# VladGavra98/SERL

Hardware: NVIDIA H100
Metric: env_steps_per_sec (higher is better)
Workload: dtype f64 plant + f32 actor

## Files before the change

serl_b200/csrc/gen/plant_rhs_common.h:

```cpp
#define PLANT_NPV 23
PLANT_PV_TABLE = {
  {0x1.6800000000000p+6, 0x0.0p+0, (1.0/0.0), (-1.0/0.0), (1.0/0.0), (-1.0/0.0), 0x1.489db496242c0p-3, 0x1.489db496242c0p-3, 0x1.489db496242c0p-3, 0x1.097333cd78a88p-1, 0x1.10eafeb224ae4p+2, 0x1.99c1db3619942p+2, 0x1.99c1db3619942p+2, 0x1.097333cd78a88p-1, 0x1.10eafeb224ae4p+2, 0x1.10eafeb224ae4p+2, 0x1.10eafeb224ae4p+2, 0x1.097333cd78a88p-1, 0x1.097333cd78a88p-1, 0x1.99c1db3619942p+2, -0x1.097333cd78a88p-1, -0x1.097333cd78a88p-1, -0x1.99c1db3619942p+2},
  {0x1.6800000000000p+6, 0x1.eb851eb851eb8p-5, 0x1.ae147ae147ae1p-1, -0x1.ae147ae147ae1p-1, 0x1.ae147ae147ae1p-1, -0x1.ae147ae147ae1p-1, 0x1.489db496242c0p-3, 0x1.489db496242c0p-3, 0x1.489db496242c0p-3, 0x1.097333cd78a88p-1, 0x1.10eafeb224ae4p+2, 0x1.99c1db3619942p+2, 0x1.99c1db3619942p+2, 0x1.097333cd78a88p-1, 0x1.10eafeb224ae4p+2, 0x1.10eafeb224ae4p+2, 0x1.10eafeb224ae4p+2, 0x1.097333cd78a88p-1, 0x1.097333cd78a88p-1, 0x1.99c1db3619942p+2, -0x1.097333cd78a88p-1, -0x1.097333cd78a88p-1, -0x1.99c1db3619942p+2},
  {0x1.6800000000000p+6, 0x0.0p+0, (1.0/0.0), (-1.0/0.0), (1.0/0.0), (-1.0/0.0), -0x1.6ec496d3b7a80p-4, -0x1.6ec496d3b7a80p-4, -0x1.6ec496d3b7a80p-4, 0x1.12e6679af1510p-2, 0x1.20eafeb224ae4p+2, 0x1.89c1db3619942p+2, 0x1.89c1db3619942p+2, 0x1.12e6679af1510p-2, 0x1.20eafeb224ae4p+2, 0x1.20eafeb224ae4p+2, 0x1.20eafeb224ae4p+2, 0x1.12e6679af1510p-2, 0x1.12e6679af1510p-2, 0x1.89c1db3619942p+2, -0x1.12e6679af1510p-2, -0x1.12e6679af1510p-2, -0x1.89c1db3619942p+2},
  {0x1.6800000000000p+6, 0x0.0p+0, (1.0/0.0), (-1.0/0.0), (1.0/0.0), (-1.0/0.0), 0x1.489db496242c0p-3, 0x1.489db496242c0p-3, 0x1.489db496242c0p-3, 0x1.097333cd78a88p-1, 0x1.10eafeb224ae4p+2, 0x1.99c1db3619942p+2, 0x1.99c1db3619942p+2, 0x1.097333cd78a88p-1, 0x1.10eafeb224ae4p+2, 0x1.10eafeb224ae4p+2, 0x1.10eafeb224ae4p+2, 0x1.097333cd78a88p-1, 0x1.097333cd78a88p-1, 0x1.99c1db3619942p+2, -0x1.097333cd78a88p-1, -0x1.097333cd78a88p-1, -0x1.99c1db3619942p+2},
  {0x1.2c00000000000p+7, 0x0.0p+0, (1.0/0.0), (-1.0/0.0), (1.0/0.0), (-1.0/0.0), 0x1.489db496242c0p-3, 0x1.489db496242c0p-3, 0x1.489db496242c0p-3, 0x1.097333cd78a88p-1, 0x1.10eafeb224ae4p+2, 0x1.99c1db3619942p+2, 0x1.99c1db3619942p+2, 0x1.097333cd78a88p-1, 0x1.10eafeb224ae4p+2, 0x1.10eafeb224ae4p+2, 0x1.10eafeb224ae4p+2, 0x1.097333cd78a88p-1, 0x1.097333cd78a88p-1, 0x1.99c1db3619942p+2, -0x1.097333cd78a88p-1, -0x1.097333cd78a88p-1, -0x1.99c1db3619942p+2},
  {0x1.6800000000000p+6, 0x0.0p+0, (1.0/0.0), (-1.0/0.0), (1.0/0.0), (-1.0/0.0), 0x1.489db496242c0p-3, 0x1.489db496242c0p-3, 0x1.489db496242c0p-3, 0x1.097333cd78a88p-1, 0x1.10eafeb224ae4p+2, 0x1.99c1db3619942p+2, 0x1.99c1db3619942p+2, 0x1.097333cd78a88p-1, 0x1.10eafeb224ae4p+2, 0x1.10eafeb224ae4p+2, 0x1.10eafeb224ae4p+2, 0x1.097333cd78a88p-1, 0x1.097333cd78a88p-1, 0x1.99c1db3619942p+2, -0x1.097333cd78a88p-1, -0x1.097333cd78a88p-1, -0x1.99c1db3619942p+2},
  {0x1.6800000000000p+6, 0x0.0p+0, (1.0/0.0), (-1.0/0.0), (1.0/0.0), (-1.0/0.0), 0x1.489db496242c0p-3, 0x1.489db496242c0p-3, 0x1.489db496242c0p-3, 0x1.097333cd78a88p-1, 0x1.10eafeb224ae4p+2, 0x1.99c1db3619942p+2, 0x1.99c1db3619942p+2, 0x1.097333cd78a88p-1, 0x1.10eafeb224ae4p+2, 0x1.10eafeb224ae4p+2, 0x1.10eafeb224ae4p+2, 0x1.097333cd78a88p-1, 0x1.097333cd78a88p-1, 0x1.99c1db3619942p+2, -0x1.097333cd78a88p-1, -0x1.097333cd78a88p-1, -0x1.99c1db3619942p+2},
  {0x1.6800000000000p+6, 0x0.0p+0, (1.0/0.0), (-1.0/0.0), (1.0/0.0), (-1.0/0.0), -0x1.6ec496d3b7a80p-4, -0x1.6ec496d3b7a80p-4, -0x1.6ec496d3b7a80p-4, 0x1.097333cd78a88p-1, 0x1.10eafeb224ae4p+2, 0x1.99c1db3619942p+2, 0x1.99c1db3619942p+2, 0x1.097333cd78a88p-1, 0x1.10eafeb224ae4p+2, 0x1.10eafeb224ae4p+2, 0x1.10eafeb224ae4p+2, 0x1.097333cd78a88p-1, 0x1.097333cd78a88p-1, 0x1.99c1db3619942p+2, -0x1.097333cd78a88p-1, -0x1.097333cd78a88p-1, -0x1.99c1db3619942p+2},
};

#ifndef PLANT_RHS_COMMON_NAME
#define PLANT_RHS_COMMON_NAME plant_rhs_common
#endif
PLANT_FN void PLANT_RHS_COMMON_NAME(const real* X, const real* U, real* xdot PLANT_XARGS, const real* __restrict__ plant_pvrow)
{
    const real v0 = X[PLANT_XI(0)];
    const real v1 = X[PLANT_XI(1)];
    const real v2 = X[PLANT_XI(2)];
    const real v3 = X[PLANT_XI(3)];
    const real v4 = X[PLANT_XI(4)];
    const real va_eff = v4 - U[3];
    const real v5 = X[PLANT_XI(5)];
    const real v6 = X[PLANT_XI(6)];
    const real v7 = X[PLANT_XI(7)];
    const real v8 = X[PLANT_XI(9)];
    const real v9 = X[PLANT_XI(12)];
    const real v10 = X[PLANT_XI(15)];
    const real v11 = X[PLANT_XI(16)];
    const real v12 = X[PLANT_XI(17)];
    const real v13 = X[PLANT_XI(18)];
    const real v14 = U[0];
    const real v15 = U[1];
    const real v16 = U[2];
    const real v17 = v8 + 0x1.84db300000000p+22;
    const real v18 = 0x1.84db300000000p+22 * v8;
    const real v19 = PLANT_DIV(v18, v17);
    const bool v20 = 0x1.57c0000000000p+13 < v19;
    const real v21 = v19 - 0x1.57c0000000000p+13;
    const real v22 = PLANT_K(0) * v21;
    real v23 = 0.0; if (v20) v23 = PLANT_EXP(v22);
    const real v24 = PLANT_K(1) * v23;
    const real v25 = v17 * v17;
    const real v26 = PLANT_K(2) * v24;
    const real v27 = PLANT_DIV(PLANT_K(3), v25);
    const real v28 = v26 * PLANT_K(4);
    const real v29 = v19 * PLANT_K(5);
    const real v30 = v29 + PLANT_K(6);
    const real v31 = v30 * PLANT_K(7);
    real v32 = 0.0; if (!v20) v32 = PLANT_POW(v31, PLANT_K(8));
    const real v33 = v32 * PLANT_K(9);
    const real v34 = PLANT_K(10) * v30;
    const real v35 = PLANT_K(2) * v33;
    const real v36 = PLANT_SQRT(v34);
    const real v37 = v35 * v30;
    const real v38 = v20 ? PLANT_K(4) : v30;
    const real v39 = v20 ? v24 : v33;
    const real v40 = v20 ? v28 : v37;
    const real v41 = v20 ? PLANT_K(11) : v36;
    const real v42 = v39 * 0x1.0000000000000p-1;
    const real v43 = v42 * v3;
    const real v44 = v43 * v3;
    const real v45 = PLANT_DIV(v3, v41);
    const real v46 = PLANT_K(12) * v45;
    const real v47 = v46 * v45;
    const real v48 = v47 + 0x1.0000000000000p+0;
    const real v49 = v44 + v44;
    const real v50 = v49 * PLANT_K(13);
    const real v51 = v48 * v38;
    const real v52 = PLANT_SQRT(v50);
    const real v53 = -0x1.0000000000000p-2 * v9;
    const real v54 = v53 + v2;
    const real v55 = 0x1.0000000000000p+0 * v54;
    const real v56 = PLANT_PV(0) - v3;
    const real v57 = v56 * 0x1.0000000000000p-1;
    const bool v58 = v57 <= 0x1.0000000000000p+0;
    const real v59 = (0x0.0p+0 > v57) ? 0x0.0p+0 : v57;
    const real v60 = v58 ? v59 : 0x1.0000000000000p+0;
    const real v61 = v55 + v16;
    const real v62 = 0x1.0000000000000p+0 * v60;
    const bool v63 = v15 > PLANT_K(14);
    const bool v64 = v14 <= PLANT_K(15);
    const bool v65 = PLANT_K(16) <= v14;
    const real v66 = (PLANT_K(17) > v14) ? PLANT_K(17) : v14;
    const real v67 = v65 ? v66 : PLANT_K(17);
    const real v68 = v64 ? v67 : PLANT_K(15);
    const bool v69 = PLANT_K(18) <= v15;
    const bool v70 = v14 > PLANT_K(15);
    const real v71 = v70 ? PLANT_K(15) : v67;
    const bool v72 = v15 > PLANT_K(19);
    const bool v73 = PLANT_K(20) > v15;
    const real v74 = v73 ? PLANT_K(20) : v15;
    const real v75 = v72 ? PLANT_K(19) : v74;
    const bool v76 = PLANT_K(16) > v14;
    const real v77 = v76 ? PLANT_K(17) : v66;
    const real v78 = v64 ? v77 : PLANT_K(15);
    const real v79 = v69 ? v71 : v78;
    const real v80 = v69 ? v75 : PLANT_K(20);
    const real v81 = v63 ? v68 : v79;
    const real v82 = v63 ? PLANT_K(19) : v80;
    const bool v83 = v61 <= PLANT_K(21);
    const real v84 = (PLANT_K(22) > v61) ? PLANT_K(22) : v61;
    const real v85 = v83 ? v84 : PLANT_K(21);
    const int i86 = (PLANT_K(23) <= va_eff) + (PLANT_K(24) <= va_eff) + (PLANT_K(25) <= va_eff) + (PLANT_K(26) <= va_eff) + (PLANT_K(27) < va_eff) + (PLANT_K(28) < va_eff) + (PLANT_K(29) < va_eff) + (PLANT_K(30) < va_eff) + (PLANT_K(31) < va_eff) + (PLANT_K(32) < va_eff) + (PLANT_K(33) < va_eff) + (PLANT_K(34) < va_eff) + (PLANT_K(35) < va_eff) + (PLANT_K(36) < va_eff) + (PLANT_K(37) < va_eff) + (PLANT_K(38) < va_eff) + (PLANT_K(39) < va_eff) + (PLANT_K(40) < va_eff) + (PLANT_K(41) < va_eff) + (PLANT_K(42) < va_eff);
    const real d87 = va_eff - PLANT_TAB(T22_5c868420f9)[i86];
    const real v88 = PLANT_TAB(D21_27418f9aeb)[i86] * d87 + PLANT_TAB(D22_5dc32f41be)[i86];
    const real v89 = v52 * PLANT_K(43);
    const bool v90 = 0x1.5000000000000p+4 > v8;
    const real v91 = v90 ? v8 : 0x1.5000000000000p+4;
    const int i92 = (PLANT_K(44) < v45) + (0x1.0000000000000p-2 < v45) + (PLANT_K(45) < v45) + (PLANT_K(46) < v45) + (PLANT_K(47) < v45) + (PLANT_K(14) < v45) + (0x1.8000000000000p-1 < v45) + (PLANT_K(48) < v45) + (PLANT_K(49) < v45) + (PLANT_K(50) < v45) + (PLANT_K(51) < v45) + (PLANT_K(52) < v45) + (PLANT_K(53) < v45) + (0x1.2000000000000p+0 < v45) + (PLANT_K(54) < v45) + (PLANT_K(55) < v45) + (PLANT_K(56) < v45) + (PLANT_K(57) < v45) + (PLANT_K(58) < v45) + (PLANT_K(59) < v45);
    const real d93 = v45 - PLANT_TAB(T22_24d1897348)[i92];
    const int k94 = i92 + 22 * i86;
    const real a95 = PLANT_TAB(D484_50bc08c548)[k94] * d93 + PLANT_TAB(T484_e8c2fe5251)[k94];
    const real b96 = PLANT_TAB(D484_50bc08c548)[k94 + 22] * d93 + PLANT_TAB(T484_e8c2fe5251)[k94 + 22];
    const real v97 = (b96 - a95) * PLANT_TAB(D21_dea349b657)[i86] * d87 + a95;
    const real v98 = v97 + v88;
    real v99, v100; PLANT_SINCOS(v4, &v99, &v100);
    real v101, v102; PLANT_SINCOS(v5, &v101, &v102);
    real v103, v104; PLANT_SINCOS(v6, &v103, &v104);
    real v105, v106; PLANT_SINCOS(v7, &v105, &v106);
    const real v107 = -v101;
    const real v108 = -v99;
    const real v109 = -v105;
    const real v110 = v104 * v106;
    const real v111 = v103 * v106;
    const real v112 = v100 * v0;
    const real v113 = v99 * v2;
    const real v114 = v112 + v113;
    const real v115 = 0x1.0000000000000p+0 * v1;
    const real v116 = v108 * v0;
    const real v117 = v100 * v2;
    const real v118 = v116 + v117;
    const real v119 = v107 * v114;
    const real v120 = v102 * v115;
    const real v121 = v119 + v120;
    const real v122 = 0x1.0000000000000p+0 * v118;
    const real v123 = v3 + v3;
    const real v124 = PLANT_DIV(PLANT_K(60), v123);
    const real v125 = v124 * v114;
    const real v126 = v124 * v118;
    const real v127 = PLANT_DIV(PLANT_K(61), v3);
    const real v128 = v115 * v127;
    const real v129 = PLANT_FABS(v5);
    const real v130 = PLANT_TAB(D21_a0746084a2)[i86] * d87 + PLANT_TAB(D22_67549d2d83)[i86];
    const real v131 = v130 * v81;
    const real v132 = v98 + v131;
    const real v133 = PLANT_FABS(v82);
    const int i134 = (PLANT_K(37) < v133) + (PLANT_K(62) < v133) + (PLANT_K(63) < v133) + (PLANT_K(64) < v133);
    const real d135 = v133 - PLANT_TAB(T6_de25a72f4d)[i134];
    const int i136 = (0x0.0p+0 < va_eff) + (PLANT_K(65) < va_eff) + (PLANT_K(37) < va_eff) + (PLANT_K(66) < va_eff);
    const real d137 = va_eff - PLANT_TAB(T6_7f5bbb0b87)[i136];
    const int k138 = i134 + 6 * i136;
    const real a139 = PLANT_TAB(D36_5fc06ada40)[k138] * d135 + PLANT_TAB(T36_ddc4c6a7a6)[k138];
    const real b140 = PLANT_TAB(D36_5fc06ada40)[k138 + 6] * d135 + PLANT_TAB(T36_ddc4c6a7a6)[k138 + 6];
    const real v141 = (b140 - a139) * PLANT_TAB(D5_1484877d05)[i136] * d137 + a139;
    const real v142 = v132 + v141;
    const int i143 = (PLANT_K(67) <= v129) + (PLANT_K(68) <= v129) + (PLANT_K(69) <= v129) + (PLANT_K(70) <= v129) + (PLANT_K(71) <= v129) + (PLANT_K(72) <= v129) + (PLANT_K(73) <= v129) + (0x0.0p+0 < v129) + (PLANT_K(74) < v129) + (PLANT_K(75) < v129) + (PLANT_K(76) < v129) + (PLANT_K(77) < v129) + (PLANT_K(65) < v129) + (PLANT_K(34) < v129) + (PLANT_K(37) < v129);
    const real d144 = v129 - PLANT_TAB(T17_9fa2ca8802)[i143];
    const real v145 = PLANT_TAB(D16_9201320bd9)[i143] * d144 + PLANT_TAB(D17_443f42fa49)[i143];
    const real v146 = v142 + v145;
    const real v147 = PLANT_TAB(D21_734b69f831)[i86] * d87 + PLANT_TAB(D22_12ceebca13)[i86];
    const real v148 = v147 * v128;
    const real v149 = v146 + v148;
    const real v150 = v85 * v85;
    const int i151 = 0;
    const real d152 = va_eff - PLANT_TAB(T2_13d92abe99)[i151];
    const real v153 = PLANT_TAB(D1_7dea362b3f)[i151] * d152 + PLANT_TAB(D2_c57683ca85)[i151];
    const real v154 = v153 * v150;
    const real v155 = v149 + v154;
    const int i156 = (PLANT_K(78) < va_eff);
    const real d157 = va_eff - PLANT_TAB(T3_01314fdb74)[i156];
    const real v158 = PLANT_TAB(D2_4ae71336e4)[i156] * d157 + PLANT_TAB(D3_7420e5c3cd)[i156];
    const int i159 = (0x1.0000000000000p+0 < v91) + (0x1.0000000000000p+1 < v91) + (0x1.8000000000000p+1 < v91) + (0x1.4000000000000p+2 < v91) + (0x1.e000000000000p+2 < v91) + (0x1.4000000000000p+3 < v91) + (0x1.e000000000000p+3 < v91) + (0x1.5000000000000p+4 < v91);
    const real d160 = v91 - PLANT_TAB(T10_5ffeecef32)[i159];
    const real v161 = PLANT_TAB(D9_2bc5ba4b15)[i159] * d160 + PLANT_TAB(T10_e7bef5a0a6)[i159];
    const real v162 = v161 * v158;
    const real v163 = v162 + v155;
    const real v164 = PLANT_PV(1) + v163;
    const real v165 = PLANT_TAB(D1_7dea362b3f)[i151] * d152 + PLANT_TAB(D2_aa06ef906c)[i151];
    const int i166 = (PLANT_K(66) < v129) + (PLANT_K(79) < v129);
    const real d167 = v129 - PLANT_TAB(T4_a49e853054)[i166];
    const int i168 = (0x0.0p+0 < va_eff) + (PLANT_K(80) < va_eff);
    const real d169 = va_eff - PLANT_TAB(T4_311aef7bf7)[i168];
    const int k170 = i166 + 4 * i168;
    const real a171 = PLANT_TAB(D16_258e228c56)[k170] * d167 + PLANT_TAB(T16_b1893e863a)[k170];
    const real b172 = PLANT_TAB(D16_258e228c56)[k170 + 4] * d167 + PLANT_TAB(T16_b1893e863a)[k170 + 4];
    const real v173 = (b172 - a171) * PLANT_TAB(D3_dab4c35e82)[i168] * d169 + a171;
    const real v174 = v165 + v173;
    const real v175 = PLANT_FABS(v85);
    const bool v176 = PLANT_K(81) >= v175;
    const real v177 = v175 - PLANT_K(81);
    const real v178 = PLANT_DIV(PLANT_K(81), v175);
    const real v179 = v177 + v177;
    const real v180 = v179 + v178;
    const real v181 = v176 ? 0x1.0000000000000p+0 : v180;
    const real v182 = PLANT_TAB(D1_7dea362b3f)[i151] * d152 + PLANT_TAB(D2_ffa1c4d8e2)[i151];
    const real v183 = v85 * v182;
    const real v184 = v183 * v181;
    const real v185 = PLANT_FABS(v81);
    const real v186 = v185 + PLANT_K(82);
    const real v187 = v185 - PLANT_K(83);
    const real v188 = v187 * 0x1.0000000000000p-2;
    const real v189 = v188 + PLANT_K(83);
    const real v190 = PLANT_DIV(v189, v186);
    const bool v191 = v190 >= 0x1.0000000000000p+0;
    const real v192 = v81 * v190;
    const real v193 = v191 ? v81 : v192;
    const int i194 = 0;
    const real d195 = v45 - PLANT_TAB(T2_c209bc6c8a)[i194];
    const int k196 = i194 + 2 * i151;
    const real a197 = PLANT_TAB(D4_70bc8f4b72)[k196] * d195 + PLANT_TAB(T4_84992ec486)[k196];
    const real b198 = PLANT_TAB(D4_70bc8f4b72)[k196 + 2] * d195 + PLANT_TAB(T4_84992ec486)[k196 + 2];
    const real v199 = (b198 - a197) * PLANT_TAB(D1_82c34fc631)[i151] * d152 + a197;
    const real v200 = PLANT_TAB(D21_27418f9aeb)[i86] * d87 + PLANT_TAB(D22_5dc32f41be)[i86];
    const real v201 = v200 + v199;
    const real v202 = v201 * v193;
    const real v203 = PLANT_K(84) * va_eff;
    const real v204 = PLANT_TAB(D2_4ae71336e4)[i156] * d157 + PLANT_TAB(D3_286dee33a4)[i156];
    const real v205 = PLANT_TAB(D9_c0e9871878)[i159] * d160 + PLANT_TAB(T10_9e4b336430)[i159];
    const real v206 = v204 * v205;
    const int k207 = i92 + 22 * i86;
    const real a208 = PLANT_TAB(D484_f55d20ff5b)[k207] * d93 + PLANT_TAB(T484_d9834305ba)[k207];
    const real b209 = PLANT_TAB(D484_f55d20ff5b)[k207 + 22] * d93 + PLANT_TAB(T484_d9834305ba)[k207 + 22];
    const real v210 = (b209 - a208) * PLANT_TAB(D21_dea349b657)[i86] * d87 + a208;
    const real v211 = PLANT_TAB(D21_0345e40574)[i86] * d87 + PLANT_TAB(D22_6af401d137)[i86];
    const real v212 = v211 + v210;
    const real v213 = v212 + v202;
    const real v214 = PLANT_TAB(D21_0ac13f5409)[i86] * d87 + PLANT_TAB(D22_7e0b1c0b40)[i86];
    const real v215 = v128 * v214;
    const real v216 = 0x1.0000000000000p+0 * v215;
    const real v217 = v216 + v213;
    const real v218 = v217 + v206;
    const bool v219 = v218 > PLANT_PV(2);
    const bool v220 = PLANT_PV(3) > v218;
    const real v221 = -v218;
    const real v222 = v220 ? PLANT_PV(4) : v221;
    const real v223 = v219 ? PLANT_PV(5) : v222;
    const real v224 = -v164;
    const real v225 = v174 * v5;
    const real v226 = PLANT_TAB(D1_7dea362b3f)[i151] * d152 + PLANT_TAB(D2_07145f18e9)[i151];
    const real v227 = v226 * v82;
    const real v228 = v227 + v225;
    const real v229 = v228 + v184;
    const real v230 = PLANT_TAB(D1_7dea362b3f)[i151] * d152 + PLANT_TAB(D2_a79f0395e0)[i151];
    const real v231 = v230 * v126;
    const real v232 = v231 + v229;
    const real v233 = v102 * v224;
    const real v234 = v101 * v232;
    const real v235 = v233 + v234;
    const real v236 = v107 * v224;
    const real v237 = v102 * v232;
    const real v238 = v236 + v237;
    const real v239 = 0x1.0000000000000p+0 * v223;
    const real v240 = v100 * v224;
    const real v241 = v108 * v223;
    const real v242 = v240 + v241;
    const real v243 = 0x1.0000000000000p+0 * v232;
    const real v244 = v99 * v224;
    const real v245 = v100 * v223;
    const real v246 = v244 + v245;
    const real v247 = PLANT_TAB(D21_c55884341e)[i86] * d87 + PLANT_TAB(D22_162a73ce48)[i86];
    const real v248 = v247 * PLANT_K(85);
    const real v249 = -v248;
    const real v250 = 0x1.0000000000000p+0 * v249;
    const real v251 = v108 * v249;
    const real v252 = v100 * v249;
    const real v253 = plant_table3(PLANT_TAB(T3_b6aaf83d9e), 3, PLANT_TAB(T4_a49e853054), 4, PLANT_TAB(T3_2471e62622), 3, PLANT_TAB(T36_bb148bb123), va_eff, v129, 0x0.0p+0);
    const int i254 = (PLANT_K(80) < va_eff);
    const real d255 = va_eff - PLANT_TAB(T3_f990d51c3b)[i254];
    const real v256 = PLANT_TAB(D2_34471b910c)[i254] * d255 + PLANT_TAB(D3_c29e52317e)[i254];
    const int i257 = (0x1.d4c0000000000p+13 < v8) + (PLANT_K(86) < v8) + (PLANT_K(87) < v8) + (PLANT_K(88) < v8) + (PLANT_K(89) < v8) + (PLANT_K(90) < v8) + (PLANT_K(91) < v8);
    const real d258 = v8 - PLANT_TAB(T9_047aad83a7)[i257];
    const int i259 = (PLANT_K(12) < v45) + (PLANT_K(80) < v45) + (PLANT_K(92) < v45) + (0x1.0000000000000p-1 < v45) + (PLANT_K(93) < v45) + (PLANT_K(94) < v45) + (PLANT_K(95) < v45);
    const real d260 = v45 - PLANT_TAB(T9_f75c29d7d0)[i259];
    const int k261 = i257 + 9 * i259;
    const real a262 = PLANT_TAB(D81_37bca88d3c)[k261] * d258 + PLANT_TAB(T81_9f1b3e2ea8)[k261];
    const real b263 = PLANT_TAB(D81_37bca88d3c)[k261 + 9] * d258 + PLANT_TAB(T81_9f1b3e2ea8)[k261 + 9];
    const real v264 = (b263 - a262) * PLANT_TAB(D8_88637b0441)[i259] * d260 + a262;
    const real v265 = v264 + v256;
    const real v266 = v265 + v253;
    const int i267 = 0;
    const real d268 = va_eff - PLANT_TAB(T2_3a6d9db902)[i267];
    const real v269 = PLANT_TAB(D1_b7563f892c)[i267] * d268 + PLANT_TAB(D2_c37bb81389)[i267];
    const int k270 = i257 + 9 * i259;
    const real a271 = PLANT_TAB(D81_37bca88d3c)[k270] * d258 + PLANT_TAB(T81_adc1c56504)[k270];
    const real b272 = PLANT_TAB(D81_37bca88d3c)[k270 + 9] * d258 + PLANT_TAB(T81_adc1c56504)[k270 + 9];
    const real v273 = (b272 - a271) * PLANT_TAB(D8_88637b0441)[i259] * d260 + a271;
    const real v274 = v273 + v269;
    const real v275 = v274 * v85;
    const real v276 = PLANT_TAB(D1_7dea362b3f)[i151] * d152 + PLANT_TAB(D2_e9d6540019)[i151];
    const int k277 = i257 + 9 * i259;
    const real a278 = PLANT_TAB(D81_37bca88d3c)[k277] * d258 + PLANT_TAB(T81_26d7c50b88)[k277];
    const real b279 = PLANT_TAB(D81_37bca88d3c)[k277 + 9] * d258 + PLANT_TAB(T81_26d7c50b88)[k277 + 9];
    const real v280 = (b279 - a278) * PLANT_TAB(D8_88637b0441)[i259] * d260 + a278;
    const real v281 = v276 + v280;
    const real v282 = PLANT_TAB(D2_54ea72a61a)[i254] * d255 + PLANT_TAB(D3_0361ada254)[i254];
    const int k283 = i194 + 2 * i151;
    const real a284 = PLANT_TAB(D4_70bc8f4b72)[k283] * d195 + PLANT_TAB(T4_92800ee231)[k283];
    const real b285 = PLANT_TAB(D4_70bc8f4b72)[k283 + 2] * d195 + PLANT_TAB(T4_92800ee231)[k283 + 2];
    const real v286 = (b285 - a284) * PLANT_TAB(D1_82c34fc631)[i151] * d152 + a284;
    const real v287 = va_eff - PLANT_K(96);
    const real v288 = v287 * 0x1.0000000000000p+0;
    const real v289 = 0x1.0000000000000p+0 - v288;
    const bool v290 = v289 <= 0x1.0000000000000p+0;
    const bool v291 = 0x0.0p+0 > v289;
    const real v292 = v291 ? 0x0.0p+0 : v289;
    const real v293 = v290 ? v292 : 0x1.0000000000000p+0;
    const int i294 = (0x1.6800000000000p+6 < v89);
    const real d295 = v89 - PLANT_TAB(T3_97c4b3dfe6)[i294];
    const real v296 = PLANT_TAB(D2_3a06809fef)[i294] * d295 + PLANT_TAB(T3_0df123a5ac)[i294];
    const int i297 = (0x1.0000000000000p+0 < v45) + (PLANT_K(97) < v45) + (PLANT_K(98) < v45) + (PLANT_K(99) < v45) + (PLANT_K(100) < v45) + (0x1.4000000000000p+0 < v45) + (PLANT_K(101) < v45) + (PLANT_K(102) < v45) + (PLANT_K(103) < v45) + (PLANT_K(104) < v45) + (0x1.8000000000000p+0 < v45) + (PLANT_K(105) < v45) + (PLANT_K(106) < v45) + (PLANT_K(107) < v45) + (PLANT_K(108) < v45) + (0x1.c000000000000p+0 < v45) + (PLANT_K(109) < v45) + (PLANT_K(110) < v45) + (PLANT_K(111) < v45) + (PLANT_K(112) < v45);
    const real d298 = v45 - PLANT_TAB(T22_58e2189475)[i297];
    const int k299 = i297 + 22 * i86;
    const real a300 = PLANT_TAB(D484_a175432a9f)[k299] * d298 + PLANT_TAB(T484_560bcae58e)[k299];
    const real b301 = PLANT_TAB(D484_a175432a9f)[k299 + 22] * d298 + PLANT_TAB(T484_560bcae58e)[k299 + 22];
    const real v302 = (b301 - a300) * PLANT_TAB(D21_dea349b657)[i86] * d87 + a300;
    const real v303 = PLANT_TAB(D21_27418f9aeb)[i86] * d87 + PLANT_TAB(D22_5dc32f41be)[i86];
    const real v304 = v303 + v302;
    const real v305 = v304 * v81;
    const real v306 = v293 * v305;
    const int i307 = (0x1.2c00000000000p+6 < v89);
    const real d308 = v89 - PLANT_TAB(T3_9d3ff750a8)[i307];
    const real v309 = PLANT_TAB(D2_50641bdc5c)[i307] * d308 + PLANT_TAB(T3_0df123a5ac)[i307];
    const real v310 = v309 * v296;
    const real v311 = v310 * v306;
    const real v312 = PLANT_TAB(D21_35c8ac45ca)[i86] * d87 + PLANT_TAB(D22_62df2c5f97)[i86];
    const real v313 = PLANT_K(113) * v203;
    const real v314 = PLANT_FABS(va_eff);
    const real v315 = v314 * 0x1.4000000000000p+2;
    const real v316 = 0x1.0000000000000p+0 - v315;
    const bool v317 = 0x1.0000000000000p-2 >= v316;
    const real v318 = -v316;
    const real v319 = v317 ? -0x1.0000000000000p-2 : v318;
    const real v320 = v319 * v81;
    const real v321 = v320 * v296;
    const real v322 = PLANT_TAB(D9_195e7e60a4)[i159] * d160 + PLANT_TAB(T10_f5a661a073)[i159];
    const real v323 = PLANT_TAB(D1_50e4fa6347)[i267] * d268 + PLANT_TAB(D2_7f6b3fce9b)[i267];
    const int k324 = i257 + 9 * i259;
    const real a325 = PLANT_TAB(D81_37bca88d3c)[k324] * d258 + PLANT_TAB(T81_a7ade31227)[k324];
    const real b326 = PLANT_TAB(D81_37bca88d3c)[k324 + 9] * d258 + PLANT_TAB(T81_a7ade31227)[k324 + 9];
    const real v327 = (b326 - a325) * PLANT_TAB(D8_88637b0441)[i259] * d260 + a325;
    const real v328 = v323 + v327;
    const int k329 = i166 + 4 * i168;
    const real a330 = PLANT_TAB(D16_db8d312704)[k329] * d167 + PLANT_TAB(T16_be23e0de27)[k329];
    const real b331 = PLANT_TAB(D16_db8d312704)[k329 + 4] * d167 + PLANT_TAB(T16_be23e0de27)[k329 + 4];
    const real v332 = (b331 - a330) * PLANT_TAB(D3_dab4c35e82)[i168] * d169 + a330;
    const real v333 = v328 + v332;
    const real v334 = PLANT_TAB(D2_9bb4db9322)[i254] * d255 + PLANT_TAB(D3_cffb7989c5)[i254];
    const int k335 = i257 + 9 * i259;
    const real a336 = PLANT_TAB(D81_37bca88d3c)[k335] * d258 + PLANT_TAB(T81_1512909bd9)[k335];
    const real b337 = PLANT_TAB(D81_37bca88d3c)[k335 + 9] * d258 + PLANT_TAB(T81_1512909bd9)[k335 + 9];
    const real v338 = (b337 - a336) * PLANT_TAB(D8_88637b0441)[i259] * d260 + a336;
    const real v339 = v338 + v334;
    const real v340 = PLANT_TAB(D1_7dea362b3f)[i151] * d152 + PLANT_TAB(D2_65dd21f48d)[i151];
    const real v341 = v266 * v5;
    const real v342 = PLANT_TAB(D1_7dea362b3f)[i151] * d152 + PLANT_TAB(D2_ca9df7c311)[i151];
    const real v343 = v342 * v82;
    const real v344 = v343 + v341;
    const real v345 = v344 + v275;
    const real v346 = v126 * v282;
    const real v347 = v125 * v281;
    const real v348 = v345 + v347;
    const real v349 = v348 + v346;
    const int k350 = i92 + 22 * i86;
    const real a351 = PLANT_TAB(D484_dd2766afa8)[k350] * d93 + PLANT_TAB(T484_6eaa2a375b)[k350];
    const real b352 = PLANT_TAB(D484_dd2766afa8)[k350 + 22] * d93 + PLANT_TAB(T484_6eaa2a375b)[k350 + 22];
    const real v353 = (b352 - a351) * PLANT_TAB(D21_dea349b657)[i86] * d87 + a351;
    const real v354 = PLANT_TAB(D21_27418f9aeb)[i86] * d87 + PLANT_TAB(D22_5dc32f41be)[i86];
    const real v355 = v354 + v353;
    const real v356 = v311 + v355;
    const int i357 = 0;
    const real d358 = v175 - PLANT_TAB(T2_5a1c4bdea4)[i357];
    const int i359 = 0;
    const real d360 = v129 - PLANT_TAB(T2_3917b41baf)[i359];
    const int k361 = i357 + 2 * i359;
    const real a362 = PLANT_TAB(D4_5f878b5336)[k361] * d358 + PLANT_TAB(T4_7a12bddf1a)[k361];
    const real b363 = PLANT_TAB(D4_5f878b5336)[k361 + 2] * d358 + PLANT_TAB(T4_7a12bddf1a)[k361 + 2];
    const real v364 = (b363 - a362) * PLANT_TAB(D1_b11a293006)[i359] * d360 + a362;
    const real v365 = v364 + v356;
    const real v366 = PLANT_TAB(D16_3e9f23fbcf)[i143] * d144 + PLANT_TAB(D17_2ac31ef8e9)[i143];
    const real v367 = v128 * v312;
    const real v368 = v366 + v365;
    const real v369 = v367 + v368;
    const real v370 = PLANT_TAB(D2_4ae71336e4)[i156] * d157 + PLANT_TAB(D3_64138e8b45)[i156];
    const real v371 = v370 + v313;
    const real v372 = v371 + v321;
    const real v373 = v372 * v322;
    const real v374 = v373 + v369;
    const real v375 = PLANT_TAB(D2_23d85fa70b)[i254] * d255 + PLANT_TAB(D3_44423f8b91)[i254];
    const int k376 = i257 + 9 * i259;
    const real a377 = PLANT_TAB(D81_37bca88d3c)[k376] * d258 + PLANT_TAB(T81_6fda6fc830)[k376];
    const real b378 = PLANT_TAB(D81_37bca88d3c)[k376 + 9] * d258 + PLANT_TAB(T81_6fda6fc830)[k376 + 9];
    const real v379 = (b378 - a377) * PLANT_TAB(D8_88637b0441)[i259] * d260 + a377;
    const real v380 = v379 + v375;
    const real v381 = v380 * v82;
    const real v382 = v333 * v5;
    const real v383 = v381 + v382;
    const real v384 = PLANT_TAB(D1_7dea362b3f)[i151] * d152 + PLANT_TAB(D2_fd679980a0)[i151];
    const real v385 = PLANT_K(114) * v85;
    const real v386 = v384 * v85;
    const real v387 = v385 * v286;
    const real v388 = v386 + v383;
    const real v389 = v125 * v339;
    const real v390 = v126 * v340;
    const real v391 = v387 + v388;
    const real v392 = v391 + v389;
    const real v393 = v392 + v390;
    const real v394 = v100 * v349;
    const real v395 = v108 * v393;
    const real v396 = v394 + v395;
    const real v397 = 0x1.0000000000000p+0 * v374;
    const real v398 = v99 * v349;
    const real v399 = v100 * v393;
    const real v400 = v398 + v399;
    const real v401 = v243 * PLANT_K(115);
    const real v402 = v401 * PLANT_K(116);
    const real v403 = v243 * PLANT_PV(6);
    const real v404 = v246 * PLANT_PV(7);
    const real v405 = v242 * PLANT_K(115);
    const real v406 = v404 - v405;
    const real v407 = v406 * PLANT_K(118);
    const real v408 = 0x0.0p+0 - v403;
    const real v409 = v408 * PLANT_K(116);
    const real v410 = v322 * -0x1.0000000000000p+1;
    const real v411 = 0x1.0000000000000p+0 * v410;
    const real v412 = PLANT_K(119) * v44;
    const real v413 = v235 * v412;
    const real v414 = v238 * v412;
    const real v415 = v239 * v412;
    const real v416 = v396 + v402;
    const real v417 = v416 * v412;
    const real v418 = v397 + v407;
    const real v419 = v418 * v412;
    const real v420 = v400 + v409;
    const real v421 = v420 * v412;
    const real v422 = v252 * PLANT_PV(8);
    const real v423 = v251 * PLANT_K(115);
    const real v424 = v422 - v423;
    const real v425 = v424 * PLANT_K(118);
    const real v426 = v250 * v412;
    const real v427 = v426 * v127;
    const real v428 = v411 + v425;
    const real v429 = v428 * v412;
    const real v430 = v429 * v127;
    const real v431 = 0x1.1940000000000p+12 * v27;
    const real v432 = v40 * PLANT_K(120);
    const int i433 = (0x1.e000000000000p+4 < v10) + (0x1.4000000000000p+5 < v10) + (0x1.9000000000000p+5 < v10) + (0x1.e000000000000p+5 < v10) + (0x1.1800000000000p+6 < v10) + (0x1.4000000000000p+6 < v10) + (0x1.6800000000000p+6 < v10) + (0x1.9000000000000p+6 < v10) + (0x1.b800000000000p+6 < v10);
    const real d434 = v10 - PLANT_TAB(T11_a5c2a1bb3b)[i433];
    const int i435 = (PLANT_K(12) < v45) + (PLANT_K(92) < v45) + (PLANT_K(93) < v45) + (PLANT_K(95) < v45) + (PLANT_K(121) < v45) + (PLANT_K(122) < v45) + (PLANT_K(123) < v45) + (PLANT_K(124) < v45) + (PLANT_K(125) < v45);
    const real d436 = v45 - PLANT_TAB(T11_950e09ebe5)[i435];
    const int k437 = i433 + 11 * i435;
    const real a438 = PLANT_TAB(D121_cef40c3754)[k437] * d434 + PLANT_TAB(T121_c23389a80c)[k437];
    const real b439 = PLANT_TAB(D121_cef40c3754)[k437 + 11] * d434 + PLANT_TAB(T121_c23389a80c)[k437 + 11];
    const real v440 = (b439 - a438) * PLANT_TAB(D10_477eadeedb)[i435] * d436 + a438;
    const real v441 = v432 * v440;
    const real v442 = v441 * PLANT_K(126);
    const int i443 = (0x1.e000000000000p+4 < v11) + (0x1.4000000000000p+5 < v11) + (0x1.9000000000000p+5 < v11) + (0x1.e000000000000p+5 < v11) + (0x1.1800000000000p+6 < v11) + (0x1.4000000000000p+6 < v11) + (0x1.6800000000000p+6 < v11) + (0x1.9000000000000p+6 < v11) + (0x1.b800000000000p+6 < v11);
    const real d444 = v11 - PLANT_TAB(T11_a5c2a1bb3b)[i443];
    const int k445 = i443 + 11 * i435;
    const real a446 = PLANT_TAB(D121_cef40c3754)[k445] * d444 + PLANT_TAB(T121_c23389a80c)[k445];
    const real b447 = PLANT_TAB(D121_cef40c3754)[k445 + 11] * d444 + PLANT_TAB(T121_c23389a80c)[k445 + 11];
    const real v448 = (b447 - a446) * PLANT_TAB(D10_477eadeedb)[i435] * d436 + a446;
    const real v449 = v448 * v432;
    const real v450 = v449 * PLANT_K(126);
    const real v451 = -v442;
    const real v452 = v450 + v442;
    const real v453 = -v450;
    const real v454 = v450 * PLANT_K(127);
    const real v455 = v453 * PLANT_K(128);
    const real v456 = v451 * PLANT_K(128);
    const real v457 = v442 * PLANT_K(129);
    const real v458 = v457 + v454;
    const real v459 = v456 + v455;
    const real v460 = v100 * v452;
    const real v461 = v108 * v452;
    const real v462 = v102 * v460;
    const real v463 = v107 * v460;
    const real v464 = 0x1.0000000000000p+0 * v461;
    const real v465 = PLANT_K(130) * v452;
    const real v466 = -v465;
    const real v467 = v109 * v431;
    const real v468 = v111 * v431;
    const real v469 = v110 * v431;
    const real v470 = v100 * v467;
    const real v471 = v99 * v469;
    const real v472 = v470 + v471;
    const real v473 = 0x1.0000000000000p+0 * v468;
    const real v474 = v108 * v467;
    const real v475 = v100 * v469;
    const real v476 = v474 + v475;
    const real v477 = v102 * v472;
    const real v478 = v101 * v473;
    const real v479 = v477 + v478;
    const real v480 = v107 * v472;
    const real v481 = v102 * v473;
    const real v482 = v480 + v481;
    const real v483 = 0x1.0000000000000p+0 * v476;
    const real v484 = v102 * v3;
    const real v485 = v101 * v3;
    const real v486 = v100 * v484;
    const real v487 = 0x1.0000000000000p+0 * v485;
    const real v488 = v99 * v484;
    const real v489 = v109 * v486;
    const real v490 = v111 * v487;
    const real v491 = v489 + v490;
    const real v492 = v110 * v488;
    const real v493 = v491 + v492;
    const real v494 = -v493;
    const real v495 = PLANT_PV(9) * v105;
    const real v496 = PLANT_K(132) - v8;
    const real v497 = PLANT_PV(10) * v105;
    const real v498 = v496 + v495;
    const real v499 = PLANT_K(134) * v103;
    const real v500 = v499 + v498;
    const real v501 = PLANT_K(135) - v8;
    const real v502 = v501 - v497;
    const real v503 = PLANT_K(136) * v103;
    const real v504 = v498 + v503;
    const real v505 = PLANT_K(137) - v8;
    const real v506 = PLANT_PV(11) * v105;
    const real v507 = v505 + v506;
    const bool v508 = v507 >= PLANT_K(139);
    const real v509 = PLANT_PV(12) * v1;
    const real v510 = v509 * v106;
    const real v511 = v510 + v493;
    const real v512 = v511 * 0x1.3880000000000p+14;
    const real v513 = v512 + 0x1.9000000000000p+9;
    const bool v514 = v513 > 0x0.0p+0;
    const real v515 = v514 ? v513 : 0.0;
    const bool v516 = v507 >= 0x0.0p+0;
    const real v517 = 0x1.3880000000000p+15 * v507;
    const real v518 = v512 + v517;
    const bool v519 = v518 > 0x0.0p+0;
    const real v520 = v519 ? v518 : 0.0;
    const real v521 = v516 ? v520 : 0x0.0p+0;
    const real v522 = v508 ? v515 : v521;
    const real v523 = v104 * v109;
    const real v524 = v109 * v103;
    const real v525 = v106 * v104;
    const real v526 = v525 * v522;
// ... 214 lines not shown
    const real v741 = v413 + v462;
    const real v742 = v741 + v479;
    const real v743 = v742 + v736;
    const real v744 = v414 + v463;
    const real v745 = v744 + v482;
    const real v746 = v745 + v739;
    const real v747 = v415 + v464;
    const real v748 = v747 + v483;
    const real v749 = v748 + v740;
    const real v750 = v121 * v3;
    const real v751 = v3 * v122;
    const real v752 = 0x0.0p+0 - v750;
    const real v753 = v752 * 0x1.1940000000000p+12;
    const real v754 = v749 - v753;
    const real v755 = v751 * 0x1.1940000000000p+12;
    const real v756 = v746 - v755;
    const real v757 = v3 * v102;
    const real v758 = v3 * 0x1.1940000000000p+12;
    const real v759 = v757 * 0x1.1940000000000p+12;
    const real v760 = v759 - v427;
    const real v761 = v760 * v758;
    const real v762 = v758 * v754;
    const real v763 = v760 * v756;
    const real v764 = PLANT_K(60) * v417;
    const real v765 = PLANT_DIV(v762, v761);
    const real v766 = v764 + v700;
    const real v767 = PLANT_DIV(v763, v761);
    const real v768 = PLANT_K(60) * v421;
    const real v769 = v768 + v458;
    const real v770 = v769 + v726;
    const real v771 = PLANT_K(147) * v0;
    const real v772 = PLANT_K(148) * v2;
    const real v773 = PLANT_K(61) * v419;
    const real v774 = v772 + v771;
    const real v775 = v774 * v1;
    const real v776 = v766 * PLANT_K(149);
    const real v777 = v775 + v776;
    const real v778 = v770 * PLANT_K(150);
    const real v779 = v777 + v778;
    const real v780 = v459 + v466;
    const real v781 = v773 + v780;
    const real v782 = PLANT_K(61) * v430;
    const real v783 = v781 + v717;
    const real v784 = v782 * v765;
    const real v785 = v783 + v784;
    const real v786 = PLANT_K(151) * v785;
    const real v787 = PLANT_K(152) * v0;
    const real v788 = v2 * v787;
    const real v789 = v0 * v0;
    const real v790 = v2 * v2;
    const real v791 = PLANT_K(147) * v2;
    const real v792 = v789 - v790;
    const real v793 = PLANT_K(153) * v0;
    const real v794 = PLANT_K(150) * v766;
    const real v795 = v770 * PLANT_K(154);
    const real v796 = v792 * PLANT_K(155);
    const real v797 = v793 - v791;
    const real v798 = v797 * v1;
    const real v799 = v788 - v796;
    const real v800 = v799 + v786;
    const real v801 = v798 + v794;
    const real v802 = v801 + v795;
    const real v803 = v743 * PLANT_K(156);
    const real v804 = PLANT_DIV(v105, v106);
    const real v805 = v1 * v103;
    const real v806 = v2 * v104;
    const real v807 = v103 * v2;
    const real v808 = v104 * v1;
    const real v809 = v805 + v806;
    const real v810 = v808 - v807;
    const real v811 = v809 * v804;
    const real v812 = v811 + v0;
    const real v813 = PLANT_K(84) * v62;
    const bool v814 = v813 > 0x1.f000000000000p+5;
    const bool v815 = 0x1.b000000000000p+3 > v813;
    const real v816 = v813 - 0x1.b000000000000p+3;
    const real v817 = v816 * PLANT_K(157);
    const real v818 = v817 * 0x1.1800000000000p+5;
    const real v819 = 0x1.2000000000000p+3 + v818;
    const real v820 = v815 ? 0x1.2000000000000p+3 : v819;
    const real v821 = v814 ? 0x1.6000000000000p+5 : v820;
    const real v822 = PLANT_K(158) * v8;
    const real v823 = v822 * PLANT_K(85);
    const int i824 = (0x1.4000000000000p+3 < v821) + (0x1.e000000000000p+3 < v821) + (0x1.4000000000000p+4 < v821) + (0x1.9000000000000p+4 < v821) + (0x1.e000000000000p+4 < v821) + (0x1.1800000000000p+5 < v821) + (0x1.4000000000000p+5 < v821);
    const real d825 = v821 - PLANT_TAB(T9_1b846bfe5a)[i824];
    const int i826 = (0x1.9000000000000p+7 < v823) + (0x1.2c00000000000p+8 < v823) + (0x1.9000000000000p+8 < v823) + (0x1.e000000000000p+8 < v823) + (0x1.1800000000000p+9 < v823) + (0x1.4000000000000p+9 < v823) + (0x1.6800000000000p+9 < v823);
    const real d827 = v823 - PLANT_TAB(T9_e37bea49dd)[i826];
    const int k828 = i824 + 9 * i826;
    const real a829 = PLANT_TAB(D81_512e2aee4a)[k828] * d825 + PLANT_TAB(T81_65f9a37a64)[k828];
    const real b830 = PLANT_TAB(D81_512e2aee4a)[k828 + 9] * d825 + PLANT_TAB(T81_65f9a37a64)[k828 + 9];
    const real v831 = (b830 - a829) * PLANT_TAB(D8_e4a49c3404)[i826] * d827 + a829;
    const real v832 = v51 * PLANT_K(7);
    const bool v833 = 0x0.0p+0 > v832;
    const real v834 = -v832;
    const real v835 = PLANT_SQRT(v834);
    const real v836 = -v835;
    const real v837 = PLANT_SQRT(v832);
    const real v838 = v833 ? v836 : v837;
    const real v839 = PLANT_DIV(v831, v838);
    const int i840 = (0x1.9000000000000p+5 < v839) + (0x1.b800000000000p+5 < v839) + (0x1.e000000000000p+5 < v839) + (0x1.0400000000000p+6 < v839) + (0x1.1800000000000p+6 < v839) + (0x1.2c00000000000p+6 < v839) + (0x1.4000000000000p+6 < v839) + (0x1.5400000000000p+6 < v839) + (0x1.6800000000000p+6 < v839) + (0x1.7c00000000000p+6 < v839) + (0x1.9000000000000p+6 < v839);
    const real d841 = v839 - PLANT_TAB(T13_af740fea6b)[i840];
    const int i842 = (PLANT_K(12) < v45) + (PLANT_K(92) < v45) + (PLANT_K(93) < v45) + (PLANT_K(95) < v45) + (PLANT_K(159) < v45) + (0x1.0000000000000p+0 < v45) + (PLANT_K(98) < v45) + (PLANT_K(123) < v45) + (PLANT_K(101) < v45) + (PLANT_K(160) < v45) + (0x1.8000000000000p+0 < v45);
    const real d843 = v45 - PLANT_TAB(T13_eb1e5ad919)[i842];
    const int k844 = i840 + 13 * i842;
    const real a845 = PLANT_TAB(D169_d48756a93d)[k844] * d841 + PLANT_TAB(T169_734c4fd336)[k844];
    const real b846 = PLANT_TAB(D169_d48756a93d)[k844 + 13] * d841 + PLANT_TAB(T169_734c4fd336)[k844 + 13];
    const real v847 = (b846 - a845) * PLANT_TAB(D12_7a33282c7c)[i842] * d843 + a845;
    const real v848 = v847 - v11;
    const real v849 = v848 + v848;
    const real v850 = PLANT_DIV(v12, v838);
    const int i851 = (0x1.9000000000000p+4 < v850) + (0x1.4000000000000p+5 < v850) + (0x1.1800000000000p+6 < v850) + (0x1.7800000000000p+6 < v850);
    const real d852 = v850 - PLANT_TAB(T6_4f757d8087)[i851];
    const real v853 = PLANT_TAB(D5_5f3c1eaf32)[i851] * d852 + PLANT_TAB(T6_c180cfbfe0)[i851];
    const real v854 = v853 - v849;
    const bool v855 = v854 >= 0x0.0p+0;
    const real v856 = v855 ? v849 : v853;
    const int i857 = (0x1.9000000000000p+5 < v850) + (0x1.e000000000000p+5 < v850) + (0x1.7800000000000p+6 < v850);
    const real d858 = v850 - PLANT_TAB(T5_915a9d44dd)[i857];
    const real v859 = PLANT_TAB(D4_5c024609f2)[i857] * d858 + PLANT_TAB(T5_7017f30e5f)[i857];
    const real v860 = v856 - v859;
    const real v861 = v831 - v12;
    const bool v862 = 0x0.0p+0 > v860;
    const real v863 = v862 ? v859 : v856;
    const int i864 = 0;
    const real d865 = v831 - PLANT_TAB(T2_a8f73221a0)[i864];
    const real v866 = PLANT_TAB(D1_140792e8b7)[i864] * d865 + PLANT_TAB(T2_7d0eaebb13)[i864];
    const real v867 = v861 * v866;
    const int i868 = (0x1.4000000000000p+5 < v12) + (0x1.1800000000000p+6 < v12);
    const real d869 = v12 - PLANT_TAB(T4_dd9b4b98b4)[i868];
    const real v870 = PLANT_TAB(D3_048d12320c)[i868] * d869 + PLANT_TAB(T4_989b1deebb)[i868];
    const real v871 = v870 - v867;
    const bool v872 = 0x0.0p+0 <= v871;
    const real v873 = v872 ? v867 : v870;
    const int i874 = (0x1.9000000000000p+5 < v12) + (0x1.e000000000000p+5 < v12) + (0x1.7800000000000p+6 < v12);
    const real d875 = v12 - PLANT_TAB(T5_915a9d44dd)[i874];
    const real v876 = PLANT_TAB(D4_74dca2257a)[i874] * d875 + PLANT_TAB(T5_a1035d5bbb)[i874];
    const real v877 = v873 - v876;
    const bool v878 = 0x0.0p+0 <= v877;
    const real v879 = v878 ? v873 : v876;
    const real v880 = v847 - v10;
    const real v881 = PLANT_DIV(v13, v838);
    const real v882 = v880 + v880;
    const int i883 = (0x1.9000000000000p+4 < v881) + (0x1.4000000000000p+5 < v881) + (0x1.1800000000000p+6 < v881) + (0x1.7800000000000p+6 < v881);
    const real d884 = v881 - PLANT_TAB(T6_4f757d8087)[i883];
    const real v885 = PLANT_TAB(D5_5f3c1eaf32)[i883] * d884 + PLANT_TAB(T6_c180cfbfe0)[i883];
    const real v886 = v885 - v882;
    const bool v887 = 0x0.0p+0 <= v886;
    const real v888 = v887 ? v882 : v885;
    const int i889 = (0x1.9000000000000p+5 < v881) + (0x1.e000000000000p+5 < v881) + (0x1.7800000000000p+6 < v881);
    const real d890 = v881 - PLANT_TAB(T5_915a9d44dd)[i889];
    const real v891 = PLANT_TAB(D4_5c024609f2)[i889] * d890 + PLANT_TAB(T5_7017f30e5f)[i889];
    const real v892 = v888 - v891;
    const real v893 = v831 - v13;
    const bool v894 = 0x0.0p+0 <= v892;
    const real v895 = v894 ? v888 : v891;
    const real v896 = v893 * v866;
    const int i897 = (0x1.4000000000000p+5 < v13) + (0x1.1800000000000p+6 < v13);
    const real d898 = v13 - PLANT_TAB(T4_dd9b4b98b4)[i897];
    const real v899 = PLANT_TAB(D3_048d12320c)[i897] * d898 + PLANT_TAB(T4_989b1deebb)[i897];
    const real v900 = v899 - v896;
    const bool v901 = 0x0.0p+0 <= v900;
    const real v902 = v901 ? v896 : v899;
    const int i903 = (0x1.9000000000000p+5 < v13) + (0x1.e000000000000p+5 < v13) + (0x1.7800000000000p+6 < v13);
    const real d904 = v13 - PLANT_TAB(T5_915a9d44dd)[i903];
    const real v905 = PLANT_TAB(D4_74dca2257a)[i903] * d904 + PLANT_TAB(T5_a1035d5bbb)[i903];
    const real v906 = v902 - v905;
    const bool v907 = 0x0.0p+0 <= v906;
    const real v908 = v907 ? v902 : v905;
    xdot[PLANT_XI(0)] = v779;
    xdot[PLANT_XI(1)] = v800;
    xdot[PLANT_XI(2)] = v802;
    xdot[PLANT_XI(3)] = v803;
    xdot[PLANT_XI(4)] = v765;
    xdot[PLANT_XI(5)] = v767;
    xdot[PLANT_XI(6)] = v812;
    xdot[PLANT_XI(7)] = v810;
    xdot[PLANT_XI(9)] = v494;
    xdot[PLANT_XI(12)] = v54;
    xdot[PLANT_XI(15)] = v895;
    xdot[PLANT_XI(16)] = v863;
    xdot[PLANT_XI(17)] = v879;
    xdot[PLANT_XI(18)] = v908;
}
```

Baseline: 401.5 million.

## Replace linear comparison-sum table index searches with arithmetic guess plus one correction

Each breakpoint index search in the lookup tables used to be a sum of up to twenty double-precision comparisons. It now computes a guess arithmetically: a float affine map and clamp for uniform grids, or a popcount of a precomputed bitmask over a fine grid for non-uniform ones. A single table comparison then corrects the guess. This cuts the FP64 compare work, which is slow on this GPU, in the plant right-hand side. In exchange it adds dependent table loads and relies on the generated masks and scale factors matching the breakpoints exactly.

```diff
diff --git a/serl_b200/csrc/gen/plant_rhs_common.h b/serl_b200/csrc/gen/plant_rhs_common.h
--- a/serl_b200/csrc/gen/plant_rhs_common.h
+++ b/serl_b200/csrc/gen/plant_rhs_common.h
@@ -102,13 +102,15 @@
     const bool v83 = v61 <= PLANT_K(21);
     const real v84 = (PLANT_K(22) > v61) ? PLANT_K(22) : v61;
     const real v85 = v83 ? v84 : PLANT_K(21);
-    const int i86 = (PLANT_K(23) <= va_eff) + (PLANT_K(24) <= va_eff) + (PLANT_K(25) <= va_eff) + (PLANT_K(26) <= va_eff) + (PLANT_K(27) < va_eff) + (PLANT_K(28) < va_eff) + (PLANT_K(29) < va_eff) + (PLANT_K(30) < va_eff) + (PLANT_K(31) < va_eff) + (PLANT_K(32) < va_eff) + (PLANT_K(33) < va_eff) + (PLANT_K(34) < va_eff) + (PLANT_K(35) < va_eff) + (PLANT_K(36) < va_eff) + (PLANT_K(37) < va_eff) + (PLANT_K(38) < va_eff) + (PLANT_K(39) < va_eff) + (PLANT_K(40) < va_eff) + (PLANT_K(41) < va_eff) + (PLANT_K(42) < va_eff);
+    const int g86 = __builtin_popcount(0x7eaad555u & ((1u << (int)fminf(fmaxf(((float)va_eff - -0x1.0cb7a80000000p-4f) * 0x1.bbf7920000000p+6f, 0.0f), 31.0f)) - 1u));
+    const int i86 = g86 + ((PLANT_TAB(T22_5c868420f9)[g86 + 1] < va_eff) | ((PLANT_TAB(T22_5c868420f9)[g86 + 1] == va_eff) & (g86 < 4)));
     const real d87 = va_eff - PLANT_TAB(T22_5c868420f9)[i86];
     const real v88 = PLANT_TAB(D21_27418f9aeb)[i86] * d87 + PLANT_TAB(D22_5dc32f41be)[i86];
     const real v89 = v52 * PLANT_K(43);
     const bool v90 = 0x1.5000000000000p+4 > v8;
     const real v91 = v90 ? v8 : 0x1.5000000000000p+4;
-    const int i92 = (PLANT_K(44) < v45) + (0x1.0000000000000p-2 < v45) + (PLANT_K(45) < v45) + (PLANT_K(46) < v45) + (PLANT_K(47) < v45) + (PLANT_K(14) < v45) + (0x1.8000000000000p-1 < v45) + (PLANT_K(48) < v45) + (PLANT_K(49) < v45) + (PLANT_K(50) < v45) + (PLANT_K(51) < v45) + (PLANT_K(52) < v45) + (PLANT_K(53) < v45) + (0x1.2000000000000p+0 < v45) + (PLANT_K(54) < v45) + (PLANT_K(55) < v45) + (PLANT_K(56) < v45) + (PLANT_K(57) < v45) + (PLANT_K(58) < v45) + (PLANT_K(59) < v45);
+    const int g92 = __builtin_popcount(0x5eef54a5u & ((1u << (int)fminf(fmaxf(((float)v45 - 0x1.0860440000000p-3f) * 0x1.7e96ec0000000p+4f, 0.0f), 31.0f)) - 1u));
+    const int i92 = g92 + (PLANT_TAB(T22_24d1897348)[g92 + 1] < v45);
     const real d93 = v45 - PLANT_TAB(T22_24d1897348)[i92];
     const int k94 = i92 + 22 * i86;
     const real a95 = PLANT_TAB(D484_50bc08c548)[k94] * d93 + PLANT_TAB(T484_e8c2fe5251)[k94];
@@ -155,7 +157,8 @@
     const real b140 = PLANT_TAB(D36_5fc06ada40)[k138 + 6] * d135 + PLANT_TAB(T36_ddc4c6a7a6)[k138 + 6];
     const real v141 = (b140 - a139) * PLANT_TAB(D5_1484877d05)[i136] * d137 + a139;
     const real v142 = v132 + v141;
-    const int i143 = (PLANT_K(67) <= v129) + (PLANT_K(68) <= v129) + (PLANT_K(69) <= v129) + (PLANT_K(70) <= v129) + (PLANT_K(71) <= v129) + (PLANT_K(72) <= v129) + (PLANT_K(73) <= v129) + (0x0.0p+0 < v129) + (PLANT_K(74) < v129) + (PLANT_K(75) < v129) + (PLANT_K(76) < v129) + (PLANT_K(77) < v129) + (PLANT_K(65) < v129) + (PLANT_K(34) < v129) + (PLANT_K(37) < v129);
+    const int g143 = __builtin_popcount(0x8db5b11u & ((1u << (int)fminf(fmaxf(((float)v129 - -0x1.70e77e0000000p-3f) * 0x1.634d060000000p+6f, 0.0f), 31.0f)) - 1u));
+    const int i143 = g143 + ((PLANT_TAB(T17_9fa2ca8802)[g143 + 1] < v129) | ((PLANT_TAB(T17_9fa2ca8802)[g143 + 1] == v129) & (g143 < 7)));
     const real d144 = v129 - PLANT_TAB(T17_9fa2ca8802)[i143];
     const real v145 = PLANT_TAB(D16_9201320bd9)[i143] * d144 + PLANT_TAB(D17_443f42fa49)[i143];
     const real v146 = v142 + v145;
@@ -171,7 +174,8 @@
     const int i156 = (PLANT_K(78) < va_eff);
     const real d157 = va_eff - PLANT_TAB(T3_01314fdb74)[i156];
     const real v158 = PLANT_TAB(D2_4ae71336e4)[i156] * d157 + PLANT_TAB(D3_7420e5c3cd)[i156];
-    const int i159 = (0x1.0000000000000p+0 < v91) + (0x1.0000000000000p+1 < v91) + (0x1.8000000000000p+1 < v91) + (0x1.4000000000000p+2 < v91) + (0x1.e000000000000p+2 < v91) + (0x1.4000000000000p+3 < v91) + (0x1.e000000000000p+3 < v91) + (0x1.5000000000000p+4 < v91);
+    const int g159 = __builtin_popcount(0x8afu & ((1u << (int)fminf(fmaxf(((float)v91 - 0x1.5555560000000p-2f) * 0x1.8000000000000p-1f, 0.0f), 15.0f)) - 1u));
+    const int i159 = g159 + (PLANT_TAB(T10_5ffeecef32)[g159 + 1] < v91);
     const real d160 = v91 - PLANT_TAB(T10_5ffeecef32)[i159];
     const real v161 = PLANT_TAB(D9_2bc5ba4b15)[i159] * d160 + PLANT_TAB(T10_e7bef5a0a6)[i159];
     const real v162 = v161 * v158;
@@ -269,9 +273,11 @@
     const int i254 = (PLANT_K(80) < va_eff);
     const real d255 = va_eff - PLANT_TAB(T3_f990d51c3b)[i254];
     const real v256 = PLANT_TAB(D2_34471b910c)[i254] * d255 + PLANT_TAB(D3_c29e52317e)[i254];
-    const int i257 = (0x1.d4c0000000000p+13 < v8) + (PLANT_K(86) < v8) + (PLANT_K(87) < v8) + (PLANT_K(88) < v8) + (PLANT_K(89) < v8) + (PLANT_K(90) < v8) + (PLANT_K(91) < v8);
+    const int g257 = (int)fminf(fmaxf(((float)v8 - 0x1.b344920000000p+13f) * 0x1.e955e20000000p-12f, 0.0f), 6.0f);
+    const int i257 = g257 + (PLANT_TAB(T9_047aad83a7)[g257 + 1] < v8);
     const real d258 = v8 - PLANT_TAB(T9_047aad83a7)[i257];
-    const int i259 = (PLANT_K(12) < v45) + (PLANT_K(80) < v45) + (PLANT_K(92) < v45) + (0x1.0000000000000p-1 < v45) + (PLANT_K(93) < v45) + (PLANT_K(94) < v45) + (PLANT_K(95) < v45);
+    const int g259 = (int)fminf(fmaxf(((float)v45 - 0x1.3333340000000p-3f) * 0x1.4000000000000p+3f, 0.0f), 6.0f);
+    const int i259 = g259 + (PLANT_TAB(T9_f75c29d7d0)[g259 + 1] < v45);
     const real d260 = v45 - PLANT_TAB(T9_f75c29d7d0)[i259];
     const int k261 = i257 + 9 * i259;
     const real a262 = PLANT_TAB(D81_37bca88d3c)[k261] * d258 + PLANT_TAB(T81_9f1b3e2ea8)[k261];
@@ -309,7 +315,8 @@
     const int i294 = (0x1.6800000000000p+6 < v89);
     const real d295 = v89 - PLANT_TAB(T3_97c4b3dfe6)[i294];
     const real v296 = PLANT_TAB(D2_3a06809fef)[i294] * d295 + PLANT_TAB(T3_0df123a5ac)[i294];
-    const int i297 = (0x1.0000000000000p+0 < v45) + (PLANT_K(97) < v45) + (PLANT_K(98) < v45) + (PLANT_K(99) < v45) + (PLANT_K(100) < v45) + (0x1.4000000000000p+0 < v45) + (PLANT_K(101) < v45) + (PLANT_K(102) < v45) + (PLANT_K(103) < v45) + (PLANT_K(104) < v45) + (0x1.8000000000000p+0 < v45) + (PLANT_K(105) < v45) + (PLANT_K(106) < v45) + (PLANT_K(107) < v45) + (PLANT_K(108) < v45) + (0x1.c000000000000p+0 < v45) + (PLANT_K(109) < v45) + (PLANT_K(110) < v45) + (PLANT_K(111) < v45) + (PLANT_K(112) < v45);
+    const int g297 = (int)fminf(fmaxf(((float)v45 - 0x1.f333340000000p-1f) * 0x1.4000000000000p+4f, 0.0f), 19.0f);
+    const int i297 = g297 + (PLANT_TAB(T22_58e2189475)[g297 + 1] < v45);
     const real d298 = v45 - PLANT_TAB(T22_58e2189475)[i297];
     const int k299 = i297 + 22 * i86;
     const real a300 = PLANT_TAB(D484_a175432a9f)[k299] * d298 + PLANT_TAB(T484_560bcae58e)[k299];
@@ -445,9 +452,11 @@
     const real v430 = v429 * v127;
     const real v431 = 0x1.1940000000000p+12 * v27;
     const real v432 = v40 * PLANT_K(120);
-    const int i433 = (0x1.e000000000000p+4 < v10) + (0x1.4000000000000p+5 < v10) + (0x1.9000000000000p+5 < v10) + (0x1.e000000000000p+5 < v10) + (0x1.1800000000000p+6 < v10) + (0x1.4000000000000p+6 < v10) + (0x1.6800000000000p+6 < v10) + (0x1.9000000000000p+6 < v10) + (0x1.b800000000000p+6 < v10);
+    const int g433 = (int)fminf(fmaxf(((float)v10 - 0x1.9000000000000p+4f) * 0x1.99999a0000000p-4f, 0.0f), 8.0f);
+    const int i433 = g433 + (PLANT_TAB(T11_a5c2a1bb3b)[g433 + 1] < v10);
     const real d434 = v10 - PLANT_TAB(T11_a5c2a1bb3b)[i433];
-    const int i435 = (PLANT_K(12) < v45) + (PLANT_K(92) < v45) + (PLANT_K(93) < v45) + (PLANT_K(95) < v45) + (PLANT_K(121) < v45) + (PLANT_K(122) < v45) + (PLANT_K(123) < v45) + (PLANT_K(124) < v45) + (PLANT_K(125) < v45);
+    const int g435 = __builtin_popcount(0x36a5u & ((1u << (int)fminf(fmaxf(((float)v45 - 0x1.4320fe0000000p-3f) * 0x1.7af2860000000p+3f, 0.0f), 15.0f)) - 1u));
+    const int i435 = g435 + (PLANT_TAB(T11_950e09ebe5)[g435 + 1] < v45);
     const real d436 = v45 - PLANT_TAB(T11_950e09ebe5)[i435];
     const int k437 = i433 + 11 * i435;
     const real a438 = PLANT_TAB(D121_cef40c3754)[k437] * d434 + PLANT_TAB(T121_c23389a80c)[k437];
@@ -455,7 +464,8 @@
     const real v440 = (b439 - a438) * PLANT_TAB(D10_477eadeedb)[i435] * d436 + a438;
     const real v441 = v432 * v440;
     const real v442 = v441 * PLANT_K(126);
-    const int i443 = (0x1.e000000000000p+4 < v11) + (0x1.4000000000000p+5 < v11) + (0x1.9000000000000p+5 < v11) + (0x1.e000000000000p+5 < v11) + (0x1.1800000000000p+6 < v11) + (0x1.4000000000000p+6 < v11) + (0x1.6800000000000p+6 < v11) + (0x1.9000000000000p+6 < v11) + (0x1.b800000000000p+6 < v11);
+    const int g443 = (int)fminf(fmaxf(((float)v11 - 0x1.9000000000000p+4f) * 0x1.99999a0000000p-4f, 0.0f), 8.0f);
+    const int i443 = g443 + (PLANT_TAB(T11_a5c2a1bb3b)[g443 + 1] < v11);
     const real d444 = v11 - PLANT_TAB(T11_a5c2a1bb3b)[i443];
     const int k445 = i443 + 11 * i435;
     const real a446 = PLANT_TAB(D121_cef40c3754)[k445] * d444 + PLANT_TAB(T121_c23389a80c)[k445];
@@ -836,9 +846,11 @@
     const real v821 = v814 ? 0x1.6000000000000p+5 : v820;
     const real v822 = PLANT_K(158) * v8;
     const real v823 = v822 * PLANT_K(85);
-    const int i824 = (0x1.4000000000000p+3 < v821) + (0x1.e000000000000p+3 < v821) + (0x1.4000000000000p+4 < v821) + (0x1.9000000000000p+4 < v821) + (0x1.e000000000000p+4 < v821) + (0x1.1800000000000p+5 < v821) + (0x1.4000000000000p+5 < v821);
+    const int g824 = (int)fminf(fmaxf(((float)v821 - 0x1.e000000000000p+2f) * 0x1.99999a0000000p-3f, 0.0f), 6.0f);
+    const int i824 = g824 + (PLANT_TAB(T9_1b846bfe5a)[g824 + 1] < v821);
     const real d825 = v821 - PLANT_TAB(T9_1b846bfe5a)[i824];
-    const int i826 = (0x1.9000000000000p+7 < v823) + (0x1.2c00000000000p+8 < v823) + (0x1.9000000000000p+8 < v823) + (0x1.e000000000000p+8 < v823) + (0x1.1800000000000p+9 < v823) + (0x1.4000000000000p+9 < v823) + (0x1.6800000000000p+9 < v823);
+    const int g826 = (int)fminf(fmaxf(((float)v823 - 0x1.3955560000000p+7f) * 0x1.7a17a20000000p-7f, 0.0f), 6.0f);
+    const int i826 = g826 + (PLANT_TAB(T9_e37bea49dd)[g826 + 1] < v823);
     const real d827 = v823 - PLANT_TAB(T9_e37bea49dd)[i826];
     const int k828 = i824 + 9 * i826;
     const real a829 = PLANT_TAB(D81_512e2aee4a)[k828] * d825 + PLANT_TAB(T81_65f9a37a64)[k828];
@@ -852,9 +864,11 @@
     const real v837 = PLANT_SQRT(v832);
     const real v838 = v833 ? v836 : v837;
     const real v839 = PLANT_DIV(v831, v838);
-    const int i840 = (0x1.9000000000000p+5 < v839) + (0x1.b800000000000p+5 < v839) + (0x1.e000000000000p+5 < v839) + (0x1.0400000000000p+6 < v839) + (0x1.1800000000000p+6 < v839) + (0x1.2c00000000000p+6 < v839) + (0x1.4000000000000p+6 < v839) + (0x1.5400000000000p+6 < v839) + (0x1.6800000000000p+6 < v839) + (0x1.7c00000000000p+6 < v839) + (0x1.9000000000000p+6 < v839);
+    const int g840 = (int)fminf(fmaxf(((float)v839 - 0x1.7c00000000000p+5f) * 0x1.99999a0000000p-3f, 0.0f), 10.0f);
+    const int i840 = g840 + (PLANT_TAB(T13_af740fea6b)[g840 + 1] < v839);
     const real d841 = v839 - PLANT_TAB(T13_af740fea6b)[i840];
-    const int i842 = (PLANT_K(12) < v45) + (PLANT_K(92) < v45) + (PLANT_K(93) < v45) + (PLANT_K(95) < v45) + (PLANT_K(159) < v45) + (0x1.0000000000000p+0 < v45) + (PLANT_K(98) < v45) + (PLANT_K(123) < v45) + (PLANT_K(101) < v45) + (PLANT_K(160) < v45) + (0x1.8000000000000p+0 < v45);
+    const int g842 = __builtin_popcount(0x77a5u & ((1u << (int)fminf(fmaxf(((float)v45 - 0x1.40da740000000p-3f) * 0x1.713b140000000p+3f, 0.0f), 15.0f)) - 1u));
+    const int i842 = g842 + (PLANT_TAB(T13_eb1e5ad919)[g842 + 1] < v45);
     const real d843 = v45 - PLANT_TAB(T13_eb1e5ad919)[i842];
     const int k844 = i840 + 13 * i842;
     const real a845 = PLANT_TAB(D169_d48756a93d)[k844] * d841 + PLANT_TAB(T169_734c4fd336)[k844];
```

After: 408.7 million, median of 6. 1.02x the previous value.
